# YaoTiancheng/DirectComputeRayTracing

Hardware: AMD Instinct MI355X
Metric: Mrays/s and ms/spp at 1920x1080, 8-bounce wavefront (higher is better)
Workload: dtype f32; 1 GPU; cornell_box_obj 1920x1080, 1733 spp (1 spp/step, film stripes across 1 GPU(s)), 8 bounces, wavefront, point light; spp=1733, max_bounce=8, streams_per_gpu=3, snapshot_spp=1733, parallelism=single GPU, 3 concurrent pipelines per GPU (cost-balanced bands), partition=balanced, interleave=False, bands_per_rank=3, rays=48252902736

## Files before the change

directcomputeraytracing_amd/csrc/device/kernels.h:

```cpp
#pragma once

#include "dbsdf.h"

namespace dcrt {
namespace dev {

constexpr uint32_t kFlagIdle = 0x80000000u;
constexpr uint32_t kFlagShadowRayHit = 0x40000000u;
constexpr uint32_t kFlagTerminate = 0x20000000u;
constexpr uint32_t kFlagDelta = 0x10000000u;
constexpr uint32_t kFlagFirst = 0x08000000u;
constexpr uint32_t kFlagShadowPending = 0x04000000u;
constexpr uint32_t kFlagShadowResolved = 0x02000000u;
constexpr uint32_t kFlagIdleFrom = 0x40000000u;
constexpr uint32_t kEpochMask = 0x3FFFFFFFu;
DEV uint32_t idle_from(uint32_t epoch) { return kFlagIdleFrom | (epoch & kEpochMask); }
DEV bool slot_idle(uint32_t flags, uint32_t epoch)
{
    return (flags & kFlagIdle) != 0u || ((flags & kFlagIdleFrom) != 0u && ((epoch - flags) & kEpochMask) < (kEpochMask >> 1));
}
constexpr uint32_t kBlockW = 8, kBlockH = 8;
#ifndef DCRT_CONTROL_BLOCK
#define DCRT_CONTROL_BLOCK 256
#endif
constexpr uint32_t kControlBlock = DCRT_CONTROL_BLOCK;
static_assert(kControlBlock % 64 == 0 && kControlBlock <= 960, "CONTROL workgroup: whole waves, at most 15");

constexpr uint32_t kShards = 8;
constexpr uint32_t kShardStride = 64;
constexpr uint32_t kQExt = 0, kQShadow = 1, kQFinish = 2, kQueues = 3;
#ifndef DCRT_FIN_SHARDS
#define DCRT_FIN_SHARDS 8
#endif
constexpr uint32_t kFinShards = DCRT_FIN_SHARDS;
constexpr uint32_t kCounterWords = 2 * kShards + kFinShards;
constexpr uint32_t kVirtualWord = kCounterWords;
constexpr uint32_t kNoPixel = 0xFFFFFFFFu;
constexpr uint32_t kDrainedWord = kCounterWords + 1;
constexpr uint32_t kInlineShadowWord = kCounterWords + 2;
constexpr uint32_t kLastRayWord = kInlineShadowWord + kShards;
constexpr uint32_t kCounterLines = kLastRayWord + kShards;
constexpr uint32_t kEpochLine = kCounterLines;
constexpr uint32_t kEntryFirst = 0x80000000u;

struct Counters {
    uint32_t w[(kCounterLines + 1) * kShardStride];
// ... 165 lines not shown
}

struct F3 {
    float x, y, z;
};
struct alignas(4) F4u {
    float x, y, z, w;
};

template <typename T>
DEV T& slot(T* base, uint32_t i)
{
    return *(T*)((char*)base + (uint64_t)(i * (uint32_t)sizeof(T)));
}

template <typename T>
DEV T& sample_at(T* base, uint32_t i)
{
    return *(T*)((char*)base + (uint64_t)i * (uint64_t)sizeof(T));
}
typedef float GlobalF2 __attribute__((ext_vector_type(2)));
typedef float GlobalF4 __attribute__((ext_vector_type(4)));
DEV void store_global(float2* base, uint32_t i, float2 v)
{
    const GlobalF2 x = {v.x, v.y};
    *(__attribute__((address_space(1))) GlobalF2*)((uintptr_t)base + (uint64_t)i * 8u) = x;
}
DEV void store_global(float4* base, uint32_t i, float4 v)
{
    const GlobalF4 x = {v.x, v.y, v.z, v.w};
    *(__attribute__((address_space(1))) GlobalF4*)((uintptr_t)base + (uint64_t)i * 16u) = x;
}

struct PathStateA {
    uint4 rng;
    float4 lsrMisc;
};
struct PathStateB {
    float4 thr;
    float4 liLsr;
};
struct FinishRec {
    float4 liLsr;
    float4 lsrSlot;
};
constexpr uint32_t kFinishEarly = 1u;
constexpr uint32_t kDestFinish = 0x80000000u;

struct PathPool {
    float4* hit;
    float4* shRec;
    uint32_t* pixel;
    uint32_t* flags;
    float* extOpacity;
    float* shadowOpacity;
    float4* extRec;
    const float4* extPrevRec;
    PathStateA* stateA;
    PathStateB* stateB;
    const PathStateA* stateAPrev;
    const PathStateB* stateBPrev;
    uint32_t* shadowHit;
    const uint32_t* shadowHitPrev;
    uint32_t* shadowQueue;
    FinishRec* finRec;
    const FinishRec* finPrevRec;
    uint32_t* finHit;
    const uint32_t* finHitPrev;
    uint32_t size;
    uint32_t recCap;
    uint32_t finCap;
};
template <typename T>
DEV T& state_at(T* base, uint32_t q) { static_assert(sizeof(T) == 32, "state halves are 32 B"); return *(T*)((char*)base + (uint64_t)(q * 32u)); }

struct Film {
    float2* samplePosition;
    float4* sampleValue;
    uint4* debugRng;
    float4* accum;
    const uint32_t* rowY;
    const uint32_t* rowOwned;
    const uint32_t* blockList;
    uint32_t width, height, rowCount;
};

struct SampleOut {
    float2* samplePosition;
    float4* sampleValue;
    uint4* debugRng;
    uint32_t* rowRays;
};

DEV float2 pixel_sample(const FrameConstants& fc, uint32_t p)
{
    const uint32_t W = fc.resolution[0], wh = W * fc.resolution[1];
    const uint32_t image = p / wh, local = p - image * wh;
    const uint32_t py = local / W, px = local - py * W;
    Rng r = rng_init(px, py, image_seed(fc, image));
    const float psx = next1(r);
    const float psy = next1(r);
    return make_float2(psx, psy);
}

template <bool RAY>
DEV Rng new_path(const FrameConstants& fc, uint32_t p, V3* o, V3* d)
{
// ... 31 lines not shown
```

directcomputeraytracing_amd/csrc/device/kernels_impl.h:

```cpp
#include "kernels.h"

namespace dcrt {
namespace dev {

#ifdef DCRT_PHASE_CLOCKS
__device__ unsigned long long g_phaseClk[24];
#define DCRT_PHASE_INIT unsigned long long clk_[6] = {0, 0, 0, 0, 0, 0}; unsigned long long tP_ = __builtin_amdgcn_s_memtime()
#define DCRT_PHASE(i) do { const unsigned long long t_ = __builtin_amdgcn_s_memtime(); clk_[i] += t_ - tP_; tP_ = t_; } while (0)
#define DCRT_PHASE_COUNT(i) (++clk_[i])
#define DCRT_PHASE_FLUSH() do { if ((threadIdx.x & 63u) == 0) for (int i_ = 0; i_ < 6; ++i_) atomicAdd(&g_phaseClk[i_], clk_[i_]); } while (0)
#define DCRT_MCLK_INIT unsigned long long mclk_[8] = {0, 0, 0, 0, 0, 0, 0, 0}; unsigned long long mT_ = __builtin_amdgcn_s_memtime()
#define DCRT_MCLK(i) do { const unsigned long long t_ = __builtin_amdgcn_s_memtime(); mclk_[i] += t_ - mT_; mT_ = t_; } while (0)
#define DCRT_MCLK_FLUSH(items) do { mclk_[7] += (items); if ((threadIdx.x & 63u) == 0) for (int i_ = 0; i_ < 8; ++i_) atomicAdd(&g_phaseClk[8 + i_], mclk_[i_]); } while (0)
#define DCRT_MCLK_PARAMS , unsigned long long (&mclk_)[8], unsigned long long& mT_
#define DCRT_MCLK_ARGS , mclk_, mT_
#else
#define DCRT_MCLK_PARAMS
#define DCRT_MCLK_ARGS
#define DCRT_MCLK_INIT do {} while (0)
#define DCRT_MCLK(i) do {} while (0)
#define DCRT_MCLK_FLUSH(items) do {} while (0)
#define DCRT_PHASE_INIT do {} while (0)
#define DCRT_PHASE(i) do {} while (0)
#define DCRT_PHASE_COUNT(i) do {} while (0)
// ... 297 lines not shown
            want = __hip_atomic_load(cursor, __ATOMIC_RELAXED, __HIP_MEMORY_SCOPE_AGENT) < shardBlocks;
        uint32_t bslot, unused;
        block_append2(false, cursor, want, cursor, sm, &unused, &bslot);
        claimed = (uint32_t)__shfl((int)bslot, 0, 64);
        got = __shfl((int)want, 0, 64) != 0 && claimed < shardBlocks;
    }
    const uint32_t block = shard + claimed * kShards;
    bool newPath = false;
    V3 o = mk(0.0f, 0.0f, 0.0f), d = mk(0.0f, 0.0f, 0.0f);
    Rng rng;
    rng.s0 = rng.s1 = rng.s2 = rng.s3 = 0u;
    if (got) {
        uint32_t px = 0, py = 0, image = 0;
        if (block_pixel(*fc, film, block, lane, &px, &py, &image)) {
            rng = rng_init(px, py, image_seed(*fc, image));
            const float psx = next1(rng), psy = next1(rng);
            const float fsx = (psx + (float)px) / (float)fc->resolution[0];
            const float fsy = (psy + (float)py) / (float)fc->resolution[1];
            const float a0 = next1(rng), a1 = next1(rng), a2 = next1(rng);
            generate_ray(*fc, fsx, fsy, a0, a1, a2, &o, &d);
            if (fc->features & DCRT_FEATURE_ALLOW_ANYHIT) pool.extOpacity[tid] = next1(rng);
            pool.pixel[tid] = image * (film.width * film.height) + py * film.width + px;
            pool.flags[tid] = 0u;
            newPath = true;
        }
    }
    uint32_t eslot, unused;
    block_append2(newPath, qctr(cnt, kQExt, shard), false, qctr(cnt, kQExt, shard), sm + 32, &eslot, &unused);
    if (newPath) {
        const uint32_t q = shard * pool.recCap + eslot;
        float4* r = ext_rec(pool.extRec, q);
        r[0] = make_float4(o.x, o.y, o.z, 0.0f);
        r[1] = make_float4(d.x, d.y, d.z, asf(tid));
        PathStateA& st = state_at(pool.stateA, q);
        st.rng = make_uint4(rng.s0, rng.s1, rng.s2, rng.s3);
        st.lsrMisc = make_float4(0.0f, 0.0f, asf(kFlagDelta | kFlagFirst), asf(tid));
    }
    }
}

template <uint32_t CAPS, bool FRAMES = false>
__device__ __forceinline__ void shade_path(const DeviceScene& sc, const FrameConstants& fc, const HitRecord& hit, V3 dir, Rng& rng,
                                           uint32_t& flags, float4& thr, const F3& li, V3& T, V3& L, V3& lsr, bool& terminate,
                                           bool& hasShadow, V3& nO, V3& nD, float4& sO, V3& sD, float& extOpacity,
                                           float& shadowOpacity DCRT_MCLK_PARAMS)
{
    const uint32_t bounce = flags & 0xFFu;
    const uint32_t features = fc.features;
    const bool vndf = (features & DCRT_FEATURE_GGX_SAMPLE_VNDF) != 0;
    const bool hasHit = hit.t != inf();
    Intersection it;
    it.lightIndex = DCRT_LIGHT_INDEX_INVALID; it.triangleIndex = 0;
    it.geometryNormal = mk(0.0f, 0.0f, 0.0f);
    if (hasHit) hit_to_intersection<CAPS, FRAMES>(sc, hit, it);
    DCRT_MCLK(1);
    T = mk(thr.x, thr.y, thr.z);
    L = mk(li.x, li.y, li.z);
    {
        const uint32_t lightIndex = hasHit ? it.lightIndex : fc.envLightIndex;
        const bool visible = (features & DCRT_FEATURE_LIGHT_VISIBLE) != 0;
        if (visible ? lightIndex != DCRT_LIGHT_INDEX_INVALID : (bounce > 0 && lightIndex != DCRT_LIGHT_INDEX_INVALID)) {
            V3 radiance; float lightPdf;
            evaluate_light<CAPS>(sc, lightIndex, it.triangleIndex, it.geometryNormal, dir, hit.t, fc.lightCount, &radiance, &lightPdf);
            if (lightPdf > 0.0f) {
                const float weight = !(flags & kFlagDelta) ? power_heuristic(thr.w, lightPdf) : 1.0f;
                L = L + T * radiance * weight;
            }
        }
    }
// ... 134 lines not shown
    DCRT_MCLK_INIT;
    uint32_t itemsDone = 0;
    uint32_t round = 0;
    uint32_t doneFlag = kFlagIdle;
    if constexpr (EARLY) doneFlag = (uint32_t)__builtin_amdgcn_readfirstlane((int)idle_from(epoch_of(cnt) + 2u));
    for (uint32_t base = blockIdx.x * blockDim.x; base < count; base += gridDim.x * blockDim.x) {
    const uint32_t i = base + threadIdx.x;
    bool active = i < count;
    uint32_t newPixel = kNoPixel;
    if (virt && active) {
        newPixel = slot(pool.pixel, i);
        active = newPixel != kNoPixel;
    }
    bool terminate = false, hasShadow = false, ends = false, last = false;
    uint32_t path = 0, pix = 0;
    float4 sample = make_float4(0.0f, 0.0f, 0.0f, 0.0f);
    float2* outPos = nullptr;
    float4* outVal = nullptr;
    V3 nO = mk(0.0f, 0.0f, 0.0f), nD = mk(0.0f, 0.0f, 0.0f);
    float4 sO = make_float4(0.0f, 0.0f, 0.0f, 0.0f);
    V3 sD = mk(0.0f, 0.0f, 0.0f);
    uint32_t pathFlags = 0;
    float4 sThr = make_float4(0.0f, 0.0f, 0.0f, 0.0f);
    V3 sT = mk(0.0f, 0.0f, 0.0f), sL = mk(0.0f, 0.0f, 0.0f), sLsr = mk(0.0f, 0.0f, 0.0f);
    uint4 sRng = make_uint4(0u, 0u, 0u, 0u);
    if (active) {
        ++itemsDone;
        const float4 h4 = pool.hit[2 * i], hd = pool.hit[2 * i + 1];
        HitRecord hit;
        hit.t = h4.x; hit.u = h4.y; hit.v = h4.z; hit.tri = asu(h4.w); hit.inst = asu(hd.w);
        const V3 dir = mk(hd.x, hd.y, hd.z);
        Rng rng;
        uint32_t flags;
        float4 thr, l4, l2;
        bool shadowHit = false;
        if (virt) {
            V3 unusedO, unusedD;
            rng = new_path<false>(fcv, newPixel, &unusedO, &unusedD);
            path = i;
            flags = kFlagDelta;
            thr = make_float4(1.0f, 1.0f, 1.0f, 0.0f);
            l4 = make_float4(0.0f, 0.0f, 0.0f, 0.0f);
            l2 = make_float4(0.0f, 0.0f, 0.0f, 0.0f);
        } else {
            const uint32_t q = qpos(pool.recCap, qm, i);
            const PathStateA& ps = state_at(pool.stateAPrev, q);
            const PathStateB& psB = state_at(pool.stateBPrev, q);
            const uint4 r4 = ps.rng;
            l2 = ps.lsrMisc;
            const float4 bThr = psB.thr, bLi = psB.liLsr;
            uint32_t shRaw = 0u;
            if constexpr (FUSED) {
                if (__ballot((asu(l2.z) & kFlagShadowPending) != 0u) != 0ull) shRaw = pool.shadowHitPrev[q];
            } else {
                shRaw = pool.shadowHitPrev[q];
            }
            rng.s0 = r4.x; rng.s1 = r4.y; rng.s2 = r4.z; rng.s3 = r4.w;
            path = asu(l2.w);
            flags = asu(l2.z);
            const bool first = (flags & kFlagFirst) != 0u;
            thr = first ? make_float4(1.0f, 1.0f, 1.0f, 0.0f) : bThr;
            l4 = first ? make_float4(0.0f, 0.0f, 0.0f, 0.0f) : bLi;
            shadowHit = (flags & kFlagShadowResolved) != 0u || ((flags & kFlagShadowPending) != 0u && shRaw != 0u);
            flags &= ~(kFlagFirst | kFlagShadowPending | kFlagShadowResolved);
        }
        F3 li{l4.x, l4.y, l4.z};
        {
            const F3 lsr0{l4.w, l2.x, l2.y};
            li.x = li.x + (!shadowHit ? lsr0.x : 0.0f);
            li.y = li.y + (!shadowHit ? lsr0.y : 0.0f);
            li.z = li.z + (!shadowHit ? lsr0.z : 0.0f);
        }
        uint32_t out = path;
        asm volatile("" : "+v"(out));
        float extOpacity = 0.0f, shadowOpacity = 0.0f;
        V3 T, L, lsr;
        DCRT_MCLK(0);
        shade_path<CAPS, SCENE_LDS == 1 && !caps_any_scene(CAPS)>(sc, fcv, hit, dir, rng, flags, thr, li, T, L, lsr, terminate, hasShadow, nO, nD, sO, sD,
                         extOpacity, shadowOpacity DCRT_MCLK_ARGS);
        DCRT_MCLK(4);
        if (fcv.features & DCRT_FEATURE_ALLOW_ANYHIT) {
            if (!terminate) slot(pool.extOpacity, out) = extOpacity;
            if (hasShadow) slot(pool.shadowOpacity, out) = shadowOpacity;
        }
        ends = terminate && !hasShadow;
        if constexpr (EARLY) {
            const uint32_t mode = sc.earlyFinish;
            last = !terminate && (flags & 0xFFu) > fcv.maxBounce && mode != 0u && (mode != 2u || (path & 1u) == 0u) &&
                   (fcv.features & DCRT_FEATURE_ALLOW_ANYHIT) == 0u;
        }
        if constexpr (PROBE) {
            uint32_t* rowRays = sampleOut->rowRays;
            const uint32_t p = virt ? newPixel : slot(pool.pixel, out);
            const uint32_t W = fcv.resolution[0], wh = W * fcv.resolution[1];
            atomicAdd(&rowRays[(p % wh) / W], hasShadow ? 2u : 1u);
        }
        pathFlags = flags;
        sThr = thr;
        sT = T;
        sL = L;
        sLsr = lsr;
        sRng = make_uint4(rng.s0, rng.s1, rng.s2, rng.s3);
        if (ends || terminate || last) {
            const SampleOut so = *sampleOut;
            if (ends || last || so.debugRng) pix = slot(pool.pixel, out);
            if (ends || last) {
                sample = make_float4(L.x + 0.0f, L.y + 0.0f, L.z + 0.0f, 0.0f);
                outPos = so.samplePosition;
                outVal = so.sampleValue;
            }
            if (so.debugRng) sample_at(so.debugRng, pix) = make_uint4(rng.s0, rng.s1, rng.s2, rng.s3);
        }
    }
    bool inlined = false, occluded = false;
    if constexpr (FUSED) {
        const V3 sInv = inv_dir(sD);
        inlined = active && hasShadow && cells_finite(sInv) && (path & fcv.shadowInlineMask) == 0u;
        if (inlined)
            occluded = cells_occluded_cached(si.cells, si.res, mk(sO.x, sO.y, sO.z), sD, sO.w, sInv,
                                             (fcv.features & DCRT_FEATURE_WATERTIGHT) != 0, cellNodes, cellTris, cellLeaves);
        inlineRays += (uint32_t)__popcll(__ballot(inlined));
    }
    const bool queued = active && hasShadow && !inlined;
    DCRT_MCLK(5);
    uint32_t es, ss;
    const bool done = last && (!hasShadow || inlined);
    if (done) {
        sample.x = (sL.x + (!occluded ? sLsr.x : 0.0f)) + 0.0f;
        sample.y = (sL.y + (!occluded ? sLsr.y : 0.0f)) + 0.0f;
        sample.z = (sL.z + (!occluded ? sLsr.z : 0.0f)) + 0.0f;
    }
    const bool fin = active && ((terminate && hasShadow) || (last && !done));
    uint32_t fb;
    uint32_t lastBase = 0u, lastRank = 0u;
    if constexpr (EARLY) {
        const unsigned long long lm = __ballot(last);
        if (lm != 0ull) {
            lastRank = __builtin_amdgcn_mbcnt_hi((uint32_t)(lm >> 32), __builtin_amdgcn_mbcnt_lo((uint32_t)lm, 0u));
            const unsigned long long both = (unsigned long long)__popcll(lm) | ((unsigned long long)__popcll(__ballot(done)) << 32);
            if ((threadIdx.x & 63u) == 0u) lastBase = (uint32_t)atomicAdd(last_ctr(cnt, shard), both);
        }
    }
    block_append3(active && !terminate && !last, qctr(cnt, kQExt, shard), queued, qctr(cnt, kQShadow, shard),
                  fin, qctr(cnt, kQFinish, fshard), sm + (round & 1u) * 48u, &es, &ss, &fb);
    DCRT_MCLK(6);
    if constexpr (EARLY) lastBase = (uint32_t)__builtin_amdgcn_readfirstlane((int)lastBase);
    const uint32_t qNext = shard * pool.recCap + es;
    const uint32_t fPos = fshard * pool.finCap + fb;
    asm volatile("" ::"v"(pix));
    if (ends || done) {
        store_global(outPos, pix, pixel_sample(fcv, pix));
        store_global(outVal, pix, sample);
        slot(pool.flags, path) = done ? doneFlag : kFlagIdle;
    }
    if (last) {
        float4* r = ext_rec(pool.extRec, shard * pool.recCap + (pool.recCap - 1u - (lastBase + lastRank)));
        r[0] = make_float4(nO.x, nO.y, nO.z, 0.0f);
        r[1] = make_float4(nD.x, nD.y, nD.z, asf(path));
    }
    if (active && !terminate && !last) {
        float4* r = ext_rec(pool.extRec, qNext);
        r[0] = make_float4(nO.x, nO.y, nO.z, 0.0f);
        r[1] = make_float4(nD.x, nD.y, nD.z, asf(path));
        PathStateA& st = state_at(pool.stateA, qNext);
        PathStateB& stB = state_at(pool.stateB, qNext);
        st.rng = sRng;
        stB.thr = make_float4(sT.x, sT.y, sT.z, sThr.w);
        stB.liLsr = make_float4(sL.x, sL.y, sL.z, sLsr.x);
        st.lsrMisc = make_float4(sLsr.y, sLsr.z, asf(pathFlags | (queued ? kFlagShadowPending : 0u) | (occluded ? kFlagShadowResolved : 0u)), asf(path));
    }
    if (fin) {
        FinishRec& fr = pool.finRec[fPos];
        fr.liLsr = make_float4(sL.x, sL.y, sL.z, sLsr.x);
        fr.lsrSlot = make_float4(sLsr.y, sLsr.z, asf(path), asf(last ? kFinishEarly : 0u));
        if (inlined) pool.finHit[fPos] = occluded ? 1u : 0u;
    }
    if (queued) {
        const uint32_t sq = shard * pool.recCap + ss;
        float4* r = ext_rec(pool.shRec, sq);
        r[0] = sO;
        r[1] = make_float4(sD.x, sD.y, sD.z, asf(terminate || last ? (fPos | kDestFinish) : qNext));
        if (fcv.features & DCRT_FEATURE_ALLOW_ANYHIT) slot(pool.shadowQueue, sq) = path;
    }
    DCRT_MCLK(2);
    ++round;
    }
    if constexpr (FUSED) {
        if ((threadIdx.x & 63u) == 0u && inlineRays) atomicAdd(&inlineTotal, inlineRays);
        __syncthreads();
        if (threadIdx.x == 0 && inlineTotal) atomicAdd(&cnt->w[(kInlineShadowWord + shard) * kShardStride], inlineTotal);
    }
    DCRT_MCLK_FLUSH(itemsDone);
    (void)itemsDone;
}

#ifndef DCRT_CAST_WAVES_PER_EU
#define DCRT_CAST_WAVES_PER_EU 5
#endif
#if DCRT_CAST_WAVES_PER_EU > 0
#define DCRT_CAST_OCCUPANCY __attribute__((amdgpu_waves_per_eu(DCRT_CAST_WAVES_PER_EU, 8)))
#else
#define DCRT_CAST_OCCUPANCY
// ... 646 lines not shown
    }
    extern __shared__ uint32_t stackMem[];
    scene_cache_load(sc, stackMem, block_shift());
    if (blockIdx.x == 0 && threadIdx.x == 0) {
        cnt->w[kDrainedWord * kShardStride] = 1u;
        g->prevLive = 0u;
    }
    const bool watertight = (fc.features & DCRT_FEATURE_WATERTIGHT) != 0;
    const bool f2b = (fc.features & DCRT_FEATURE_NO_FRONT_TO_BACK) == 0;
    uint32_t* lds = stackMem + threadIdx.x;
    const uint32_t shift = block_shift();
    const SampleOut so = *sampleOut;
    uint32_t extRays = 0, shadowRays = 0;
    const uint32_t waves = gridDim.x * (blockDim.x >> 6);
    const uint32_t wave = blockIdx.x * (blockDim.x >> 6) + (threadIdx.x >> 6);
    for (uint32_t w = (threadIdx.x & 63u) * waves + wave; w < nExt + nFin; w += 64u * waves) {
        if (w >= nExt) {
            const uint32_t f = qpos(pool.finCap, fm, w - nExt);
            const FinishRec fr = pool.finRec[f];
            const bool shadowHit = pool.finHit[f] != 0u;
            const uint32_t path = asu(fr.lsrSlot.z);
            F3 li{fr.liLsr.x, fr.liLsr.y, fr.liLsr.z};
            const F3 lsr{fr.liLsr.w, fr.lsrSlot.x, fr.lsrSlot.y};
            li.x = li.x + (!shadowHit ? lsr.x : 0.0f);
            li.y = li.y + (!shadowHit ? lsr.y : 0.0f);
            li.z = li.z + (!shadowHit ? lsr.z : 0.0f);
            const uint32_t p = slot(pool.pixel, path);
            sample_at(so.samplePosition, p) = pixel_sample(fc, p);
            sample_at(so.sampleValue, p) = make_float4(li.x, li.y, li.z, 0.0f);
            slot(pool.flags, path) = kFlagIdle;
            continue;
        }
        const uint32_t q = qpos(pool.recCap, qe, w);
        const PathStateA ps = state_at(pool.stateA, q);
        const float4 h4 = pool.hit[2 * w], hd = pool.hit[2 * w + 1];
        HitRecord hit;
        hit.t = h4.x; hit.u = h4.y; hit.v = h4.z; hit.tri = asu(h4.w); hit.inst = asu(hd.w);
        V3 dir = mk(hd.x, hd.y, hd.z);
        Rng rng;
        rng.s0 = ps.rng.x; rng.s1 = ps.rng.y; rng.s2 = ps.rng.z; rng.s3 = ps.rng.w;
        const uint32_t path = asu(ps.lsrMisc.w);
        uint32_t flags = asu(ps.lsrMisc.z);
        const bool first = (flags & kFlagFirst) != 0u;
        float4 thr = make_float4(1.0f, 1.0f, 1.0f, 0.0f), l4 = make_float4(0.0f, 0.0f, 0.0f, 0.0f);
        if (!first) {
            const PathStateB psB = state_at(pool.stateB, q);
            thr = psB.thr;
            l4 = psB.liLsr;
        }
        bool shadowHit = (flags & kFlagShadowResolved) != 0u || ((flags & kFlagShadowPending) ? pool.shadowHit[q] != 0u : false);
        flags &= ~(kFlagFirst | kFlagShadowPending | kFlagShadowResolved);
        F3 li{l4.x, l4.y, l4.z};
        V3 lsr0 = mk(l4.w, ps.lsrMisc.x, ps.lsrMisc.y);
        for (;;) {
            li.x = li.x + (!shadowHit ? lsr0.x : 0.0f);
            li.y = li.y + (!shadowHit ? lsr0.y : 0.0f);
            li.z = li.z + (!shadowHit ? lsr0.z : 0.0f);
            bool terminate = false, hasShadow = false;
            V3 T, L, lsr, nO = mk(0.0f, 0.0f, 0.0f), nD = nO, sD = nO;
            float4 sO = make_float4(0.0f, 0.0f, 0.0f, 0.0f);
            float extOpacity = 0.0f, shadowOpacity = 0.0f;
            DCRT_MCLK_INIT;
            shade_path<CAPS>(sc, fc, hit, dir, rng, flags, thr, li, T, L, lsr, terminate, hasShadow, nO, nD, sO, sD,
                             extOpacity, shadowOpacity DCRT_MCLK_ARGS);
            shadowHit = false;
            if (hasShadow) {
                HitRecord sh;
                shadowHit = trace_full<true, false>(sc, mk(sO.x, sO.y, sO.z), sD, sO.w, watertight, f2b, 0.0f, lds, shift, &sh);
                ++shadowRays;
            }
            if (terminate) {
                const uint32_t p = slot(pool.pixel, path);
                sample_at(so.samplePosition, p) = pixel_sample(fc, p);
                sample_at(so.sampleValue, p) = make_float4(L.x + (!shadowHit ? lsr.x : 0.0f), L.y + (!shadowHit ? lsr.y : 0.0f),
                                                           L.z + (!shadowHit ? lsr.z : 0.0f), 0.0f);
                if (so.debugRng) sample_at(so.debugRng, p) = make_uint4(rng.s0, rng.s1, rng.s2, rng.s3);
                slot(pool.flags, path) = kFlagIdle;
                break;
            }
            if (!trace_full<false, false>(sc, nO, nD, inf(), watertight, f2b, 0.0f, lds, shift, &hit)) {
                hit.t = inf(); hit.u = 0.0f; hit.v = 0.0f; hit.tri = 0u; hit.inst = 0u;
            }
            ++extRays;
            dir = nD;
            thr = make_float4(T.x, T.y, T.z, thr.w);
            li = F3{L.x, L.y, L.z};
            lsr0 = lsr;
        }
    }
    const unsigned long long e = wave_sum(extRays), sr = wave_sum(shadowRays);
// ... 1035 lines not shown
```

directcomputeraytracing_amd/csrc/device/tracer.hip:

```cpp
#include <hip/hip_runtime.h>
#include <hip/hip_ext.h>

#include <dlfcn.h>

#include <algorithm>
#include <cmath>
#include <cstdio>
#include <cstdlib>
#include <cstring>
#include <map>
#include <mutex>
#include <string>
#include <type_traits>
#include <limits>
#include <vector>

#include "../../../include/dcrt.h"
#include "../host/bvh_layout.h"
#include "../host/film_rows.h"
#include "kernels_impl.h"

namespace dcrt {
void SetLastError(const std::string& s);
int CheckFilterParams(const dcrt_filter_params& f);
// ... 353 lines not shown
        d->triFrames = triFrames;
        d->ldsFrames = lds.frames ? 1u : 0u;
        d->envProb = envProb;
        d->envRowCdf = envRowCdf;
        d->envMarginal = envMarginal;
        d->earlyFinish = earlyFinish;
    }
    bool BakedEquals(const MaterialPlan& o) const
    {
        return caps == o.caps && mode == o.mode && materials == o.materials && lights == o.lights && lds.shading == o.lds.shading &&
               lds.rows == o.lds.rows && lds.frames == o.lds.frames && lds.cells == o.lds.cells && tables == o.tables && drainGrid == o.drainGrid &&
               envProb == o.envProb && envRowCdf == o.envRowCdf && envMarginal == o.envMarginal && earlyFinish == o.earlyFinish;
    }
};

}

struct dcrt_tracer {
    int device = 0;
    hipStream_t stream = nullptr;
    bool ownsStream = false;
    uint32_t cuCount = 1;
    CreateKnobs knobs;
    uint32_t iterationsPerRender = kDefaultIterations;
    bool debugRng = false;
    int mode = 0;
    dcrt_output_params output{ DCRT_OUTPUT_PATH_TRACING, 20u };

    uint32_t poolSize = 0;
    uint32_t controlGrid = 0, materialGrid = 0;
    std::vector<void*> poolAllocs;
    PathPool pool{};
    float4* extRecs = nullptr;
    PathStateA* stateRecsA = nullptr;
    PathStateB* stateRecsB = nullptr;
    uint32_t* shadowHits = nullptr;
    FinishRec* finRecs = nullptr;
    uint32_t* finHits = nullptr;
    FrameConstants* dFrame = nullptr;
    Counters* dCounters = nullptr;
    Globals* dGlobals = nullptr;
    Counters* hCounters = nullptr;
    dcrt_bxdf_luts* dLuts = nullptr;

    std::vector<void*> sceneAllocs;
    bool hasScene = false;
    CastPlan plan;
    dcrt_upload_stats uploadStats{};
    MaterialPlan material;
    float* dDielRows = nullptr;
    float4* dTriFrames = nullptr;
    int envSampling = DCRT_ENV_SAMPLING_UNIFORM;
    float* dEnvProb = nullptr;
    float* dEnvRowCdf = nullptr;
    float* dEnvMarginal = nullptr;
    float envBuildMs = 0.0f;
    bool EnvTableActive() const { return hasScene && envSampling == DCRT_ENV_SAMPLING_IMPORTANCE && dEnvProb != nullptr; }
    bool FusedShadow() const
    {
        return material.lds.cells != 0u && !rowProbe && plan.Cells(instrCounters, (frame.features & DCRT_FEATURE_ALLOW_ANYHIT) != 0);
    }
    dcrt_material* dMaterials = nullptr;
    dcrt_light* dLights = nullptr;
    uint32_t* dInstanceFlags = nullptr;
    std::vector<dcrt_material> hostMaterials;
    std::vector<dcrt_light> hostLights;
    uint64_t* dCells = nullptr;
    uint32_t* dCellLeaves = nullptr;
// ... 274 lines not shown
    knobs = ReadCreateKnobs();
    if ((uint64_t)poolSize * 64u > (1ull << 32)) {
        SetLastError("path pool too large: at most 2^26 slots (32-bit pool offsets)");
        return DCRT_E_LIMIT;
    }
    const size_t P = poolSize;
    CHECKED(DeviceAlloc(&pool.hit, 2 * P, &poolAllocs));
    CHECKED(DeviceAlloc(&pool.pixel, P, &poolAllocs));
    CHECKED(DeviceAlloc(&pool.flags, P, &poolAllocs));
    CHECKED(DeviceAlloc(&pool.extOpacity, P, &poolAllocs));
    CHECKED(DeviceAlloc(&pool.shadowOpacity, P, &poolAllocs));
    static_assert(kControlBlock == 256u && kMaterialBlock == 256u, "queue capacities assume 256-slot workgroups");
    const uint32_t V = poolSize / 256u;
    {
        hipDeviceProp_t prop;
        HIPCHECK(hipGetDeviceProperties(&prop, device));
        if (prop.maxSharedMemoryPerMultiProcessor > 0) g_ldsPerCU = prop.maxSharedMemoryPerMultiProcessor;
        int cPerCU = 0, mPerCU = 0;
        HIPCHECK(hipOccupancyMaxActiveBlocksPerMultiprocessor(&cPerCU, control_kernel, (int)kControlBlock, 0));
        HIPCHECK(hipOccupancyMaxActiveBlocksPerMultiprocessor(&mPerCU, MaterialPlan{}.Kernel(false, false), (int)kMaterialBlock, 0));
        auto resident = [&](int perCU, uint32_t mul) {
            if (mul == 0) return V;
            const uint64_t r = (uint64_t)std::max(1, perCU) * (uint64_t)std::max(1, prop.multiProcessorCount) * mul;
            const uint32_t g = (uint32_t)std::max<uint64_t>(kShards, r / kShards * kShards);
            return std::min(g, V);
        };
        controlGrid = resident(cPerCU, knobs.controlGridMul);
        materialGrid = resident(mPerCU, knobs.materialGridMul);
        static_assert(kFinShards == kShards, "MATERIAL's grid is a multiple of both shard counts");
    }
    pool.recCap = std::min<uint32_t>(poolSize, 2u * ((V + kShards - 1) / kShards) * 256u);
    if ((uint64_t)pool.recCap * kShards * 32u > (1ull << 32)) { SetLastError("path pool too large for the extension-queue records"); return DCRT_E_LIMIT; }
    CHECKED(DeviceAlloc(&extRecs, (size_t)pool.recCap * kShards * 2 * 2, &poolAllocs));
    CHECKED(DeviceAlloc(&stateRecsA, (size_t)pool.recCap * kShards * 2, &poolAllocs));
    CHECKED(DeviceAlloc(&stateRecsB, (size_t)pool.recCap * kShards * 2, &poolAllocs));
    CHECKED(DeviceAlloc(&shadowHits, (size_t)pool.recCap * kShards * 2, &poolAllocs));
    CHECKED(DeviceAlloc(&pool.shRec, (size_t)pool.recCap * kShards * 2, &poolAllocs));
    CHECKED(DeviceAlloc(&pool.shadowQueue, (size_t)pool.recCap * kShards, &poolAllocs));

    pool.finCap = ((V + kFinShards - 1) / kFinShards) * kMaterialBlock;
    CHECKED(DeviceAlloc(&finRecs, (size_t)pool.finCap * kFinShards * 2, &poolAllocs));
    CHECKED(DeviceAlloc(&finHits, (size_t)pool.finCap * kFinShards * 2, &poolAllocs));
    pool.size = poolSize;
    CHECKED(DeviceAlloc(&dFrame, 1, &poolAllocs));
    CHECKED(DeviceAlloc(&dSampleOut, 1, &poolAllocs));
    CHECKED(DeviceAlloc(&dCounters, 2, &poolAllocs));
    CHECKED(DeviceAlloc(&dGlobals, 1, &poolAllocs));
    CHECKED(DeviceAlloc(&dInstr, 8, &poolAllocs));
    CHECKED(DeviceAlloc(&dLuts, 1, &poolAllocs));
    HIPCHECK(hipMemsetAsync(dCounters, 0, 2 * sizeof(Counters), stream));
    HIPCHECK(hipMemsetAsync(dGlobals, 0, sizeof(Globals), stream));
    HIPCHECK(hipMemsetAsync(dInstr, 0, 8 * sizeof(unsigned long long), stream));
    HIPCHECK(hipHostMalloc((void**)&hCounters, 2 * sizeof(Counters), hipHostMallocDefault));
    CHECKED(DeviceAlloc(&dFilter, 1, &poolAllocs));
    HIPCHECK(hipHostMalloc((void**)&hFilter, sizeof(FilterConsts), hipHostMallocDefault));
    HIPCHECK(hipHostMalloc((void**)&hStop, 8 * sizeof(uint32_t), hipHostMallocDefault));
    for (hipEvent_t& e : stopEvents) HIPCHECK(hipEventCreateWithFlags(&e, hipEventDisableTiming));
    CHECKED(BuildLuts());
    HIPCHECK(hipStreamSynchronize(stream));
    return DCRT_OK;
}

static std::mutex g_lutMutex;
static std::map<int, dcrt_bxdf_luts*> g_lutCache;

int dcrt_tracer::BuildLuts()
{
    std::lock_guard<std::mutex> lock(g_lutMutex);
// ... 861 lines not shown
    fc.maxBounce = frame.max_bounce_count;
    fc.lightCount = frame.light_count;
    fc.envLightIndex = frame.environment_light_index;
    fc.features = frame.features;
    fc.blocksX = (frame.resolution[0] + kBlockW - 1) / kBlockW;
    fc.bandCount = bandCount;
    fc.blocksPerImage = listFrame ? listCount : fc.blocksX * bandCount;
#ifndef DCRT_REFILL_GLOBAL
#define DCRT_REFILL_GLOBAL 28
#endif
    fc.refillLanes = knobs.tuneOverride || plan.allCached ? knobs.refillLanes : DCRT_REFILL_GLOBAL;
    fc.parkLanes = knobs.parkLanes;
    fc.virtualStart = knobs.virtualStart && knobs.mergedCasts && !(frame.features & DCRT_FEATURE_ALLOW_ANYHIT) ? 1u : 0u;
    fc.drainPaths = !(frame.features & DCRT_FEATURE_ALLOW_ANYHIT) && !instrCounters && !extTiming && !rowProbe ? knobs.drainPaths : 0u;
    hipLaunchKernelGGL(set_frame_kernel, dim3(1), dim3(1), 0, stream, dFrame, fc);
    const uint32_t total = fc.blocksPerImage;
    const uint32_t idleThreads = std::max<uint32_t>(poolSize, 2u * (uint32_t)(sizeof(Counters) / 4));
    hipLaunchKernelGGL(set_idle_kernel, dim3((idleThreads + 255) / 256), dim3(256), 0, stream, pool, dCounters, dGlobals, total);
    HIPCHECK(hipGetLastError());
    parity = 0;
    newImage = false;
    imageComplete = false;
    return DCRT_OK;
}

int dcrt_tracer::LaunchIteration(uint32_t par, bool timed, bool sequenced)
{
    Annotation an("Iteration", !capturing);
    Counters* cnt = dCounters + par;
    Counters* next = dCounters + (par ^ 1u);
    PathPool pool = this->pool;
    pool.extRec = extRecs + (size_t)par * kShards * pool.recCap * 2;
    pool.extPrevRec = extRecs + (size_t)(par ^ 1u) * kShards * pool.recCap * 2;
    pool.stateA = stateRecsA + (size_t)par * kShards * pool.recCap;
    pool.stateB = stateRecsB + (size_t)par * kShards * pool.recCap;
    pool.stateAPrev = stateRecsA + (size_t)(par ^ 1u) * kShards * pool.recCap;
    pool.stateBPrev = stateRecsB + (size_t)(par ^ 1u) * kShards * pool.recCap;
    pool.shadowHit = shadowHits + (size_t)par * kShards * pool.recCap;
    pool.shadowHitPrev = shadowHits + (size_t)(par ^ 1u) * kShards * pool.recCap;
    pool.finRec = finRecs + (size_t)par * kFinShards * pool.finCap;
    pool.finPrevRec = finRecs + (size_t)(par ^ 1u) * kFinShards * pool.finCap;
    pool.finHit = finHits + (size_t)par * kFinShards * pool.finCap;
    pool.finHitPrev = finHits + (size_t)(par ^ 1u) * kFinShards * pool.finCap;
    const bool opacity = (frame.features & DCRT_FEATURE_ALLOW_ANYHIT) != 0;
    const CastLaunch cast = plan.Launch(instrCounters, opacity);
    const uint32_t castBlock = plan.block, castGrid = std::min<uint32_t>((poolSize + castBlock - 1) / castBlock, cast.resident);
    hipEvent_t c0 = nullptr, c1 = nullptr, m0 = nullptr, m1 = nullptr, e0 = nullptr, e1 = nullptr;
    if (timed) CHECKED(TimedPair(kTimedControl, &c0, &c1));
    {
        Annotation a("Control", !capturing);
        Film claims = film;
        claims.blockList = sequenced && adaptive ? dBlockList : nullptr;
        hipExtLaunchKernelGGL(control_kernel, dim3(controlGrid), dim3(kControlBlock), 0, stream, c0, c1, 0, pool, claims,
                              (const FrameConstants*)dFrame, cnt, (const Counters*)next, dGlobals, (uint32_t)(film.debugRng != nullptr));
    }
    const bool fused = FusedShadow();
    ShadowInline si{};
    if (fused) si = ShadowInline{ plan.sceneFlat.nodes, plan.sceneFlat.shadowCells, plan.sceneFlat.shadowLeaves, plan.sceneFlat.cachedNodes, plan.sceneFlat.shadowRes };
    if (timed) CHECKED(TimedPair(kTimedMaterial, &m0, &m1));
    {
        Annotation a("Material", !capturing);
        hipExtLaunchKernelGGL(material.Kernel(rowProbe, fused), dim3(materialGrid), dim3(kMaterialBlock), material.LdsBytes(rowProbe, fused), stream, m0, m1, 0, pool, plan.scene,
                              (const FrameConstants*)dFrame, cnt, (const Counters*)next, (const SampleOut*)dSampleOut, si);
    }
    if (timed) CHECKED(TimedPair(kTimedCast, &e0, &e1));
    Annotation castAnnotation(knobs.mergedCasts ? "Extension + shadow ray cast" : "Extension ray cast, shadow ray cast", !capturing);
    if (knobs.mergedCasts) {
        hipExtLaunchKernelGGL(cast.kernel, dim3(castGrid), dim3(castBlock), cast.lds, stream, e0, e1, 0, pool, cast.scene,
                              (const FrameConstants*)dFrame, cnt, next, dGlobals, dInstr);
    } else {
// ... 2019 lines not shown
```

Before: 19440 Mrays/s.

## Split path state into per-field columns and load shadow radiance only when pending

Replaces the two 32-byte path-state structs with separate columns for RNG, throughput, radiance+flags, slot/first bit, and light-sample radiance. The light-sample radiance is written only when a shadow ray is queued and read only when the pending flag is set. Unoccluded contributions are now folded into the radiance in-kernel, so the shadow-resolved flag goes away. The aim is to cut state traffic per bounce. The cost is more separate memory streams and allocations, and a 4-byte slot column that may coalesce less efficiently.

```diff
diff --git a/directcomputeraytracing_amd/csrc/device/kernels.h b/directcomputeraytracing_amd/csrc/device/kernels.h
--- a/directcomputeraytracing_amd/csrc/device/kernels.h
+++ b/directcomputeraytracing_amd/csrc/device/kernels.h
@@ -9,9 +9,7 @@
 constexpr uint32_t kFlagShadowRayHit = 0x40000000u;
 constexpr uint32_t kFlagTerminate = 0x20000000u;
 constexpr uint32_t kFlagDelta = 0x10000000u;
-constexpr uint32_t kFlagFirst = 0x08000000u;
 constexpr uint32_t kFlagShadowPending = 0x04000000u;
-constexpr uint32_t kFlagShadowResolved = 0x02000000u;
 constexpr uint32_t kFlagIdleFrom = 0x40000000u;
 constexpr uint32_t kEpochMask = 0x3FFFFFFFu;
 DEV uint32_t idle_from(uint32_t epoch) { return kFlagIdleFrom | (epoch & kEpochMask); }
@@ -243,20 +241,23 @@
     *(__attribute__((address_space(1))) GlobalF4*)((uintptr_t)base + (uint64_t)i * 16u) = x;
 }
 
-struct PathStateA {
-    uint4 rng;
-    float4 lsrMisc;
-};
-struct PathStateB {
-    float4 thr;
-    float4 liLsr;
-};
 struct FinishRec {
     float4 liLsr;
     float4 lsrSlot;
 };
 constexpr uint32_t kFinishEarly = 1u;
 constexpr uint32_t kDestFinish = 0x80000000u;
+
+#ifndef DCRT_LSR_COLUMN_F4
+#define DCRT_LSR_COLUMN_F4 0
+#endif
+#if DCRT_LSR_COLUMN_F4
+using LsrCol = float4;
+DEV LsrCol lsr_col(float x, float y, float z) { return make_float4(x, y, z, 0.0f); }
+#else
+using LsrCol = F3;
+DEV LsrCol lsr_col(float x, float y, float z) { return F3{x, y, z}; }
+#endif
 
 struct PathPool {
     float4* hit;
@@ -267,10 +268,16 @@
     float* shadowOpacity;
     float4* extRec;
     const float4* extPrevRec;
-    PathStateA* stateA;
-    PathStateB* stateB;
-    const PathStateA* stateAPrev;
-    const PathStateB* stateBPrev;
+    uint4* stRng;
+    float4* stThr;
+    float4* stLiFlags;
+    uint32_t* stSlot;
+    LsrCol* stLsr;
+    const uint4* stRngPrev;
+    const float4* stThrPrev;
+    const float4* stLiFlagsPrev;
+    const uint32_t* stSlotPrev;
+    const LsrCol* stLsrPrev;
     uint32_t* shadowHit;
     const uint32_t* shadowHitPrev;
     uint32_t* shadowQueue;
@@ -283,7 +290,11 @@
     uint32_t finCap;
 };
 template <typename T>
-DEV T& state_at(T* base, uint32_t q) { static_assert(sizeof(T) == 32, "state halves are 32 B"); return *(T*)((char*)base + (uint64_t)(q * 32u)); }
+DEV T& state_at(T* base, uint32_t q)
+{
+    static_assert(sizeof(T) <= 16, "path-state columns are at most 16 B wide");
+    return *(T*)((char*)base + (uint64_t)(q * (uint32_t)sizeof(T)));
+}
 
 struct Film {
     float2* samplePosition;
diff --git a/directcomputeraytracing_amd/csrc/device/kernels_impl.h b/directcomputeraytracing_amd/csrc/device/kernels_impl.h
--- a/directcomputeraytracing_amd/csrc/device/kernels_impl.h
+++ b/directcomputeraytracing_amd/csrc/device/kernels_impl.h
@@ -353,9 +353,8 @@
         float4* r = ext_rec(pool.extRec, q);
         r[0] = make_float4(o.x, o.y, o.z, 0.0f);
         r[1] = make_float4(d.x, d.y, d.z, asf(tid));
-        PathStateA& st = state_at(pool.stateA, q);
-        st.rng = make_uint4(rng.s0, rng.s1, rng.s2, rng.s3);
-        st.lsrMisc = make_float4(0.0f, 0.0f, asf(kFlagDelta | kFlagFirst), asf(tid));
+        state_at(pool.stRng, q) = make_uint4(rng.s0, rng.s1, rng.s2, rng.s3);
+        state_at(pool.stSlot, q) = tid | kEntryFirst;
     }
     }
 }
@@ -556,8 +555,9 @@
         const V3 dir = mk(hd.x, hd.y, hd.z);
         Rng rng;
         uint32_t flags;
-        float4 thr, l4, l2;
-        bool shadowHit = false;
+        float4 thr, l4;
+        F3 lsr0{0.0f, 0.0f, 0.0f};
+        bool pending = false, shadowHit = false;
         if (virt) {
             V3 unusedO, unusedD;
             rng = new_path<false>(fcv, newPixel, &unusedO, &unusedD);
@@ -565,32 +565,35 @@
             flags = kFlagDelta;
             thr = make_float4(1.0f, 1.0f, 1.0f, 0.0f);
             l4 = make_float4(0.0f, 0.0f, 0.0f, 0.0f);
-            l2 = make_float4(0.0f, 0.0f, 0.0f, 0.0f);
         } else {
             const uint32_t q = qpos(pool.recCap, qm, i);
-            const PathStateA& ps = state_at(pool.stateAPrev, q);
-            const PathStateB& psB = state_at(pool.stateBPrev, q);
-            const uint4 r4 = ps.rng;
-            l2 = ps.lsrMisc;
-            const float4 bThr = psB.thr, bLi = psB.liLsr;
+            const uint4 r4 = state_at(pool.stRngPrev, q);
+            const uint32_t sw = state_at(pool.stSlotPrev, q);
+            const float4 bThr = state_at(pool.stThrPrev, q), bLi = state_at(pool.stLiFlagsPrev, q);
+            const bool first = (sw & kEntryFirst) != 0u;
             uint32_t shRaw = 0u;
             if constexpr (FUSED) {
-                if (__ballot((asu(l2.z) & kFlagShadowPending) != 0u) != 0ull) shRaw = pool.shadowHitPrev[q];
+                if (__ballot(!first && (asu(bLi.w) & kFlagShadowPending) != 0u) != 0ull) {
+                    shRaw = pool.shadowHitPrev[q];
+                    const LsrCol l3 = state_at(pool.stLsrPrev, q);
+                    lsr0 = F3{l3.x, l3.y, l3.z};
+                }
             } else {
                 shRaw = pool.shadowHitPrev[q];
+                const LsrCol l3 = state_at(pool.stLsrPrev, q);
+                lsr0 = F3{l3.x, l3.y, l3.z};
             }
             rng.s0 = r4.x; rng.s1 = r4.y; rng.s2 = r4.z; rng.s3 = r4.w;
-            path = asu(l2.w);
-            flags = asu(l2.z);
-            const bool first = (flags & kFlagFirst) != 0u;
+            path = sw & ~kEntryFirst;
+            flags = first ? kFlagDelta : asu(bLi.w);
             thr = first ? make_float4(1.0f, 1.0f, 1.0f, 0.0f) : bThr;
             l4 = first ? make_float4(0.0f, 0.0f, 0.0f, 0.0f) : bLi;
-            shadowHit = (flags & kFlagShadowResolved) != 0u || ((flags & kFlagShadowPending) != 0u && shRaw != 0u);
-            flags &= ~(kFlagFirst | kFlagShadowPending | kFlagShadowResolved);
+            pending = (flags & kFlagShadowPending) != 0u;
+            shadowHit = shRaw != 0u;
+            flags &= ~kFlagShadowPending;
         }
         F3 li{l4.x, l4.y, l4.z};
-        {
-            const F3 lsr0{l4.w, l2.x, l2.y};
+        if (pending) {
             li.x = li.x + (!shadowHit ? lsr0.x : 0.0f);
             li.y = li.y + (!shadowHit ? lsr0.y : 0.0f);
             li.z = li.z + (!shadowHit ? lsr0.z : 0.0f);
@@ -649,12 +652,17 @@
     DCRT_MCLK(5);
     uint32_t es, ss;
     const bool done = last && (!hasShadow || inlined);
+    const bool fin = active && ((terminate && hasShadow) || (last && !done));
+    if (!queued && !fin) {
+        sL.x = sL.x + (!occluded ? sLsr.x : 0.0f);
+        sL.y = sL.y + (!occluded ? sLsr.y : 0.0f);
+        sL.z = sL.z + (!occluded ? sLsr.z : 0.0f);
+    }
     if (done) {
-        sample.x = (sL.x + (!occluded ? sLsr.x : 0.0f)) + 0.0f;
-        sample.y = (sL.y + (!occluded ? sLsr.y : 0.0f)) + 0.0f;
-        sample.z = (sL.z + (!occluded ? sLsr.z : 0.0f)) + 0.0f;
-    }
-    const bool fin = active && ((terminate && hasShadow) || (last && !done));
+        sample.x = sL.x + 0.0f;
+        sample.y = sL.y + 0.0f;
+        sample.z = sL.z + 0.0f;
+    }
     uint32_t fb;
     uint32_t lastBase = 0u, lastRank = 0u;
     if constexpr (EARLY) {
@@ -686,12 +694,11 @@
         float4* r = ext_rec(pool.extRec, qNext);
         r[0] = make_float4(nO.x, nO.y, nO.z, 0.0f);
         r[1] = make_float4(nD.x, nD.y, nD.z, asf(path));
-        PathStateA& st = state_at(pool.stateA, qNext);
-        PathStateB& stB = state_at(pool.stateB, qNext);
-        st.rng = sRng;
-        stB.thr = make_float4(sT.x, sT.y, sT.z, sThr.w);
-        stB.liLsr = make_float4(sL.x, sL.y, sL.z, sLsr.x);
-        st.lsrMisc = make_float4(sLsr.y, sLsr.z, asf(pathFlags | (queued ? kFlagShadowPending : 0u) | (occluded ? kFlagShadowResolved : 0u)), asf(path));
+        state_at(pool.stRng, qNext) = sRng;
+        state_at(pool.stThr, qNext) = make_float4(sT.x, sT.y, sT.z, sThr.w);
+        state_at(pool.stLiFlags, qNext) = make_float4(sL.x, sL.y, sL.z, asf(pathFlags | (queued ? kFlagShadowPending : 0u)));
+        state_at(pool.stSlot, qNext) = path;
+        if (queued) state_at(pool.stLsr, qNext) = lsr_col(sLsr.x, sLsr.y, sLsr.z);
     }
     if (fin) {
         FinishRec& fr = pool.finRec[fPos];
@@ -1404,30 +1411,40 @@
             continue;
         }
         const uint32_t q = qpos(pool.recCap, qe, w);
-        const PathStateA ps = state_at(pool.stateA, q);
+        const uint4 r4 = state_at(pool.stRng, q);
+        const uint32_t sw = state_at(pool.stSlot, q);
         const float4 h4 = pool.hit[2 * w], hd = pool.hit[2 * w + 1];
         HitRecord hit;
         hit.t = h4.x; hit.u = h4.y; hit.v = h4.z; hit.tri = asu(h4.w); hit.inst = asu(hd.w);
         V3 dir = mk(hd.x, hd.y, hd.z);
         Rng rng;
-        rng.s0 = ps.rng.x; rng.s1 = ps.rng.y; rng.s2 = ps.rng.z; rng.s3 = ps.rng.w;
-        const uint32_t path = asu(ps.lsrMisc.w);
-        uint32_t flags = asu(ps.lsrMisc.z);
-        const bool first = (flags & kFlagFirst) != 0u;
+        rng.s0 = r4.x; rng.s1 = r4.y; rng.s2 = r4.z; rng.s3 = r4.w;
+        const uint32_t path = sw & ~kEntryFirst;
+        const bool first = (sw & kEntryFirst) != 0u;
+        uint32_t flags = kFlagDelta;
         float4 thr = make_float4(1.0f, 1.0f, 1.0f, 0.0f), l4 = make_float4(0.0f, 0.0f, 0.0f, 0.0f);
         if (!first) {
-            const PathStateB psB = state_at(pool.stateB, q);
-            thr = psB.thr;
-            l4 = psB.liLsr;
-        }
-        bool shadowHit = (flags & kFlagShadowResolved) != 0u || ((flags & kFlagShadowPending) ? pool.shadowHit[q] != 0u : false);
-        flags &= ~(kFlagFirst | kFlagShadowPending | kFlagShadowResolved);
+            thr = state_at(pool.stThr, q);
+            l4 = state_at(pool.stLiFlags, q);
+            flags = asu(l4.w);
+        }
+        bool addLsr = (flags & kFlagShadowPending) != 0u;
+        bool shadowHit = false;
+        V3 lsr0 = mk(0.0f, 0.0f, 0.0f);
+        if (addLsr) {
+            shadowHit = pool.shadowHit[q] != 0u;
+            const LsrCol l3 = state_at(pool.stLsr, q);
+            lsr0 = mk(l3.x, l3.y, l3.z);
+        }
+        flags &= ~kFlagShadowPending;
         F3 li{l4.x, l4.y, l4.z};
-        V3 lsr0 = mk(l4.w, ps.lsrMisc.x, ps.lsrMisc.y);
         for (;;) {
-            li.x = li.x + (!shadowHit ? lsr0.x : 0.0f);
-            li.y = li.y + (!shadowHit ? lsr0.y : 0.0f);
-            li.z = li.z + (!shadowHit ? lsr0.z : 0.0f);
+            if (addLsr) {
+                li.x = li.x + (!shadowHit ? lsr0.x : 0.0f);
+                li.y = li.y + (!shadowHit ? lsr0.y : 0.0f);
+                li.z = li.z + (!shadowHit ? lsr0.z : 0.0f);
+            }
+            addLsr = true;
             bool terminate = false, hasShadow = false;
             V3 T, L, lsr, nO = mk(0.0f, 0.0f, 0.0f), nD = nO, sD = nO;
             float4 sO = make_float4(0.0f, 0.0f, 0.0f, 0.0f);
diff --git a/directcomputeraytracing_amd/csrc/device/tracer.hip b/directcomputeraytracing_amd/csrc/device/tracer.hip
--- a/directcomputeraytracing_amd/csrc/device/tracer.hip
+++ b/directcomputeraytracing_amd/csrc/device/tracer.hip
@@ -409,8 +409,11 @@
     std::vector<void*> poolAllocs;
     PathPool pool{};
     float4* extRecs = nullptr;
-    PathStateA* stateRecsA = nullptr;
-    PathStateB* stateRecsB = nullptr;
+    uint4* stateRng = nullptr;
+    float4* stateThr = nullptr;
+    float4* stateLiFlags = nullptr;
+    uint32_t* stateSlot = nullptr;
+    LsrCol* stateLsr = nullptr;
     uint32_t* shadowHits = nullptr;
     FinishRec* finRecs = nullptr;
     uint32_t* finHits = nullptr;
@@ -751,8 +754,12 @@
     pool.recCap = std::min<uint32_t>(poolSize, 2u * ((V + kShards - 1) / kShards) * 256u);
     if ((uint64_t)pool.recCap * kShards * 32u > (1ull << 32)) { SetLastError("path pool too large for the extension-queue records"); return DCRT_E_LIMIT; }
     CHECKED(DeviceAlloc(&extRecs, (size_t)pool.recCap * kShards * 2 * 2, &poolAllocs));
-    CHECKED(DeviceAlloc(&stateRecsA, (size_t)pool.recCap * kShards * 2, &poolAllocs));
-    CHECKED(DeviceAlloc(&stateRecsB, (size_t)pool.recCap * kShards * 2, &poolAllocs));
+    static_assert(sizeof(uint4) <= 16 && sizeof(float4) <= 16 && sizeof(LsrCol) <= 16, "path-state columns: 32-bit offsets");
+    CHECKED(DeviceAlloc(&stateRng, (size_t)pool.recCap * kShards * 2, &poolAllocs));
+    CHECKED(DeviceAlloc(&stateThr, (size_t)pool.recCap * kShards * 2, &poolAllocs));
+    CHECKED(DeviceAlloc(&stateLiFlags, (size_t)pool.recCap * kShards * 2, &poolAllocs));
+    CHECKED(DeviceAlloc(&stateSlot, (size_t)pool.recCap * kShards * 2, &poolAllocs));
+    CHECKED(DeviceAlloc(&stateLsr, (size_t)pool.recCap * kShards * 2, &poolAllocs));
     CHECKED(DeviceAlloc(&shadowHits, (size_t)pool.recCap * kShards * 2, &poolAllocs));
     CHECKED(DeviceAlloc(&pool.shRec, (size_t)pool.recCap * kShards * 2, &poolAllocs));
     CHECKED(DeviceAlloc(&pool.shadowQueue, (size_t)pool.recCap * kShards, &poolAllocs));
@@ -1680,10 +1687,17 @@
     PathPool pool = this->pool;
     pool.extRec = extRecs + (size_t)par * kShards * pool.recCap * 2;
     pool.extPrevRec = extRecs + (size_t)(par ^ 1u) * kShards * pool.recCap * 2;
-    pool.stateA = stateRecsA + (size_t)par * kShards * pool.recCap;
-    pool.stateB = stateRecsB + (size_t)par * kShards * pool.recCap;
-    pool.stateAPrev = stateRecsA + (size_t)(par ^ 1u) * kShards * pool.recCap;
-    pool.stateBPrev = stateRecsB + (size_t)(par ^ 1u) * kShards * pool.recCap;
+    const size_t stCur = (size_t)par * kShards * pool.recCap, stPrev = (size_t)(par ^ 1u) * kShards * pool.recCap;
+    pool.stRng = stateRng + stCur;
+    pool.stThr = stateThr + stCur;
+    pool.stLiFlags = stateLiFlags + stCur;
+    pool.stSlot = stateSlot + stCur;
+    pool.stLsr = stateLsr + stCur;
+    pool.stRngPrev = stateRng + stPrev;
+    pool.stThrPrev = stateThr + stPrev;
+    pool.stLiFlagsPrev = stateLiFlags + stPrev;
+    pool.stSlotPrev = stateSlot + stPrev;
+    pool.stLsrPrev = stateLsr + stPrev;
     pool.shadowHit = shadowHits + (size_t)par * kShards * pool.recCap;
     pool.shadowHitPrev = shadowHits + (size_t)(par ^ 1u) * kShards * pool.recCap;
     pool.finRec = finRecs + (size_t)par * kFinShards * pool.finCap;
```

Result: no change. 19620 Mrays/s, median of 6 (+0.9%).
